# nickgreenquist/cu2rec

Hardware: AMD Instinct MI355X
Metric: ratings/sec (SGD updates/sec) (higher is better)
Workload: dtype f32

## Files before the change

### cu2rec_amd/csrc/blocksolve.hip

```cpp
#include <hip/hip_runtime.h>
#include <hip/hip_ext.h>

#include <algorithm>
#include <atomic>
#include <cmath>
#include <cstdlib>
#include <limits>
#include <mutex>
#include <string>
#include <utility>
#include <vector>

#include "blocksolve.hpp"
#include "hip_check.hpp"
#include "sgd_device.hpp"

namespace cu2rec {

namespace {

using namespace dev;

constexpr int kB = kBsLinks;
constexpr int kTabAdel = 0, kTabCdel = kBsTableStride, kTabApow = 2 * kBsTableStride, kTabCpow = 3 * kBsTableStride;
constexpr int kH = 32;
constexpr int kMS = 36;

typedef float f32x16 __attribute__((ext_vector_type(16)));
typedef float f32x4 __attribute__((ext_vector_type(4)));
typedef float f32x2 __attribute__((ext_vector_type(2)));
__device__ __forceinline__ f32x4 lds4(const float4 *p) { return *reinterpret_cast<const f32x4 *>(p); }
__device__ __forceinline__ f32x2 lo2(f32x4 v) { return __builtin_shufflevector(v, v, 0, 1); }
__device__ __forceinline__ f32x2 hi2(f32x4 v) { return __builtin_shufflevector(v, v, 2, 3); }
__device__ __forceinline__ f32x2 fma2(f32x2 a, f32x2 b, f32x2 c) { return __builtin_elementwise_fma(a, b, c); }
__device__ __forceinline__ f32x2 dup2(float v) { return f32x2{v, v}; }
typedef unsigned int u32x2 __attribute__((ext_vector_type(2)));

__device__ __forceinline__ unsigned ld_agent(const unsigned *p) {
    return __hip_atomic_load(p, __ATOMIC_RELAXED, __HIP_MEMORY_SCOPE_AGENT);
}
__device__ __forceinline__ unsigned long long ld_agent(const unsigned long long *p) {
    return __hip_atomic_load(p, __ATOMIC_RELAXED, __HIP_MEMORY_SCOPE_AGENT);
}

__device__ __forceinline__ float row_pair_sum(float v) {
    const u32x2 r = __builtin_amdgcn_permlane16_swap(__float_as_uint(v), __float_as_uint(v), false, false);
    return __uint_as_float(r.x) + __uint_as_float(r.y);
}

__device__ __forceinline__ float half_sum(float v) {
    const u32x2 r = __builtin_amdgcn_permlane32_swap(__float_as_uint(v), __float_as_uint(v), false, false);
    return __uint_as_float(r.x) + __uint_as_float(r.y);
}

__device__ __forceinline__ float lane_value(float v, int lane) {
    return __int_as_float(__builtin_amdgcn_readlane(__float_as_int(v), lane));
}

__device__ __forceinline__ int acc_row(int reg, int h) { return (reg & 3) + 8 * (reg >> 2) + 4 * h; }

__device__ __forceinline__ float4 zero4() { return make_float4(0.f, 0.f, 0.f, 0.f); }

__global__ void bs_tables_kernel(SgdHyper h, float *__restrict__ t) {
    const int k = threadIdx.x;
    if (k > 2 * kB) return;
    const double a = 1.0 - static_cast<double>(h.lr) * static_cast<double>(h.q_reg);
    const double c = 1.0 - static_cast<double>(h.lr) * static_cast<double>(h.ib_reg);
    double ak = 1.0, ck = 1.0;
    for (int i = 0; i < k; ++i) {
        ak *= a;
        ck *= c;
    }
    t[kTabAdel + k] = static_cast<float>(1.0 - ak);
    t[kTabCdel + k] = static_cast<float>(1.0 - ck);
    t[kTabApow + k] = static_cast<float>(ak);
    t[kTabCpow + k] = static_cast<float>(ck);
}

__device__ __forceinline__ int lower_bound_key(const uint32_t *__restrict__ keys, int n, uint32_t target) {
    int lo = 0, hi = n;
    while (lo < hi) {
        const int mid = (lo + hi) >> 1;
        if (keys[mid] < target) lo = mid + 1; else hi = mid;
    }
    return lo;
}

__global__ __launch_bounds__(256) void bs_plan_kernel(const uint32_t *__restrict__ keys, int n_active, int n_hot,
                                                      int item_bits, int max_blocks, const int *__restrict__ item_of_rank,
                                                      int *__restrict__ chain_begin, BsChainDesc *__restrict__ chains,
                                                      BsBlockDesc *__restrict__ blocks, int *__restrict__ walk_begin, size_t stride) {
    __shared__ int s_part[256];
    const int b = blockIdx.x, tid = threadIdx.x;
    const uint32_t *kb = keys + static_cast<size_t>(b) * stride;
    int *cb = chain_begin + static_cast<size_t>(b) * (n_hot + 1);
    BsChainDesc *cd = chains + static_cast<size_t>(b) * max(n_hot, 1);
    BsBlockDesc *bd = blocks + static_cast<size_t>(b) * max_blocks;
    for (int r = tid; r <= n_hot; r += 256) cb[r] = lower_bound_key(kb, n_active, static_cast<uint32_t>(r));
    __syncthreads();
    if (tid == 0) walk_begin[b] = cb[n_hot];
    const int per = (n_hot + 255) / 256;
    const int r0 = min(tid * per, n_hot), r1 = min(r0 + per, n_hot);
    int mine = 0;
    for (int r = r0; r < r1; ++r) mine += (cb[r + 1] - cb[r] + kB - 1) / kB;
    s_part[tid] = mine;
    __syncthreads();
    __shared__ int s_total;
    if (tid == 0) {
        int run = 0;
        for (int t = 0; t < 256; ++t) {
            const int v = s_part[t];
            s_part[t] = run;
            run += v;
        }
        s_total = run;
    }
    __syncthreads();
    int off = s_part[tid];
    for (int r = r0; r < r1; ++r) {
        const int begin = cb[r], len = cb[r + 1] - begin;
        cd[r] = BsChainDesc{begin, len, off, item_of_rank[r]};
        const int nb = (len + kB - 1) / kB;
        for (int m = 0; m < nb; ++m) bd[off + m] = BsBlockDesc{begin + kB * m, min(kB, len - kB * m), r, m};
        off += nb;
    }
    for (int g = s_total + tid; g < max_blocks; g += 256) bd[g] = BsBlockDesc{0, 0, 0, 0};
}

__device__ __forceinline__ bool chain_is_lookahead(const BsIteration &it, int chain, const BsChainDesc &cd) {
    const int nblk = (cd.len + kB - 1) / kB;
    return chain < it.la_ranks && nblk >= 2 && cd.blk0 + nblk <= it.la_cap;
}

__device__ __forceinline__ void gram_cross_block(const SgdArgs &a, const BsIteration &it, int g, float4 *smem) {
    const BsBlockDesc bd = it.blocks[g];
    if (bd.n_valid == 0 || bd.m == 0 || !chain_is_lookahead(it, bd.chain, it.chains[bd.chain])) return;
    const int wave = threadIdx.x >> 6, lane = threadIdx.x & 63, k = lane & 31, h = lane >> 5;
    const int rt = wave >> 1, ct = wave & 1;
    const int nslots = a.nslots, RS = nslots | 1, S0 = (nslots + 1) >> 1;
    float4 *tile_c = smem, *tile_p = smem + kB * RS;
    {
        const int xc = static_cast<int>(it.vals[bd.pos0 + min(lane, bd.n_valid - 1)] >> 32);
        const int xp = static_cast<int>(it.vals[bd.pos0 - kB + lane] >> 32);
        const int rsub = lane >> 3, cs = lane & 7;
        const int nch = (nslots + 7) >> 3;
        for (int c0 = 0; c0 < nch; c0 += 2) {
            float4 vc[2][2], vp[2][2];
#pragma unroll
            for (int pp = 0; pp < 2; ++pp) {
                const int src_lane = 16 * wave + 8 * pp + rsub;
                const float4 *sc = reinterpret_cast<const float4 *>(a.P + static_cast<size_t>(__shfl(xc, src_lane)) * a.ldp);
                const float4 *sp = reinterpret_cast<const float4 *>(a.P + static_cast<size_t>(__shfl(xp, src_lane)) * a.ldp);
#pragma unroll
                for (int c = 0; c < 2; ++c) {
                    vc[pp][c] = sc[min(8 * (c0 + c) + cs, nslots - 1)];
                    vp[pp][c] = sp[min(8 * (c0 + c) + cs, nslots - 1)];
                }
            }
#pragma unroll
            for (int pp = 0; pp < 2; ++pp) {
                const int row = 16 * wave + 8 * pp + rsub;
#pragma unroll
                for (int c = 0; c < 2; ++c) {
                    const int slot = 8 * (c0 + c) + cs;
                    if (slot < nslots) {
                        tile_c[row * RS + slot] = row < bd.n_valid ? vc[pp][c] : zero4();
                        tile_p[row * RS + slot] = vp[pp][c];
                    }
                }
            }
        }
    }
    __syncthreads();
    f32x16 acc;
#pragma unroll
    for (int i = 0; i < 16; ++i) acc[i] = 0.f;
    {
        const float4 *ra = tile_c + (kH * rt + k) * RS, *rb = tile_p + (kH * ct + k) * RS;
        for (int c = 0; c < S0; c += 2) {
            float4 va[2], vb[2];
#pragma unroll
            for (int i = 0; i < 2; ++i) {
                const int slot = h * S0 + c + i;
                const bool ok = c + i < S0 && slot < nslots;
                const float4 t0 = ra[min(slot, nslots - 1)], t1 = rb[min(slot, nslots - 1)];
                va[i] = ok ? t0 : zero4();
                vb[i] = ok ? t1 : zero4();
            }
#pragma unroll
            for (int i = 0; i < 2; ++i) {
                const float pa[4] = {va[i].x, va[i].y, va[i].z, va[i].w}, pb[4] = {vb[i].x, vb[i].y, vb[i].z, vb[i].w};
#pragma unroll
                for (int e = 0; e < 4; ++e) acc = __builtin_amdgcn_mfma_f32_32x32x2f32(pa[e], pb[e], acc, 0, 0, 0);
            }
        }
    }
    const float lr = a.h.lr;
    float *dst = it.Nbuf + static_cast<size_t>(g) * kBsCrossFloats;
    const int j = kH * ct + k;
#pragma unroll
    for (int reg = 0; reg < 16; ++reg) {
        const int i = kH * rt + acc_row(reg, h);
        const float fd = static_cast<float>(kB - 1 + i - j);
        const float v = lr * (__builtin_amdgcn_exp2f(fd * it.log2c) + __builtin_amdgcn_exp2f(fd * it.log2a) * acc[reg]);
        dst[i * kB + j] = i < bd.n_valid ? v : 0.f;
    }
    __syncthreads();
}

constexpr int kGramTabFloats = 2 * kB;
__host__ __device__ inline size_t gram_tile_float4s(int nslots) { return static_cast<size_t>(kB) * (nslots | 1); }

__device__ __forceinline__ void gram_block(const SgdArgs &a, const BsIteration &it, int g, float4 *bs_smem) {
    const int wave = threadIdx.x >> 6, lane = threadIdx.x & 63;
    const BsBlockDesc bd = it.blocks[g];
    if (bd.n_valid == 0) return;
    const int nslots = a.nslots, RS = nslots | 1;
    float4 *tile = bs_smem;
    float *Ms = reinterpret_cast<float *>(bs_smem);
    float *Ns = Ms + 2 * kH * kMS;
    float *tab = Ms + max(static_cast<int>(4 * gram_tile_float4s(nslots)), 5 * kH * kMS);
    float *basev = tab + kGramTabFloats;
    const bool mine = lane < bd.n_valid;
    const uint64_t val = it.vals[bd.pos0 + min(lane, bd.n_valid - 1)];
    const int x = static_cast<int>(val >> 32);
    if (wave == 3) {
        const float r0 = (__uint_as_float(static_cast<uint32_t>(val)) - a.global_bias) - a.user_bias[x];
        basev[lane] = mine ? r0 : 0.f;
        tab[lane] = it.tables[kTabApow + lane];
        tab[kB + lane] = it.tables[kTabCpow + lane];
    }
    const int rsub = lane >> 3, cs = lane & 7;
    const int nch = (nslots + 7) >> 3;
    for (int c0 = 0; c0 < nch; c0 += 4) {
        float4 v[2][4];
#pragma unroll
        for (int pp = 0; pp < 2; ++pp) {
            const int xr = __shfl(x, 16 * wave + 8 * pp + rsub);
            const float4 *src = reinterpret_cast<const float4 *>(a.P + static_cast<size_t>(xr) * a.ldp);
#pragma unroll
            for (int c = 0; c < 4; ++c) v[pp][c] = src[min(8 * (c0 + c) + cs, nslots - 1)];
        }
#pragma unroll
        for (int pp = 0; pp < 2; ++pp) {
            const int row = 16 * wave + 8 * pp + rsub;
#pragma unroll
            for (int c = 0; c < 4; ++c) {
                const int slot = 8 * (c0 + c) + cs;
                if (slot < nslots) tile[row * RS + slot] = row < bd.n_valid ? v[pp][c] : zero4();
            }
        }
    }
    __syncthreads();
    const int k = lane & 31, h = lane >> 5;
    f32x16 acc;
#pragma unroll
    for (int i = 0; i < 16; ++i) acc[i] = 0.f;
    if (wave < 3) {
        const int S0 = (nslots + 1) >> 1;
        const float4 *ra = tile + (wave == 1 ? kH + k : k) * RS, *rb = tile + (wave == 0 ? k : kH + k) * RS;
        for (int c = 0; c < S0; c += 2) {
            float4 va[2], vb[2];
#pragma unroll
            for (int i = 0; i < 2; ++i) {
                const int slot = h * S0 + c + i;
                const bool ok = c + i < S0 && slot < nslots;
                const float4 t0 = ra[min(slot, nslots - 1)], t1 = rb[min(slot, nslots - 1)];
                va[i] = ok ? t0 : zero4();
                vb[i] = ok ? t1 : zero4();
            }
#pragma unroll
            for (int i = 0; i < 2; ++i) {
                const float pa[4] = {va[i].x, va[i].y, va[i].z, va[i].w}, pb[4] = {vb[i].x, vb[i].y, vb[i].z, vb[i].w};
#pragma unroll
                for (int e = 0; e < 4; ++e) acc = __builtin_amdgcn_mfma_f32_32x32x2f32(pa[e], pb[e], acc, 0, 0, 0);
            }
        }
    }
    __syncthreads();
    if (wave < 3) {
        const float lr = a.h.lr;
        const int K = (wave == 0 ? 0 : kH) + k;
        const int J0 = (wave == 1 ? kH : 0) + 4 * h;
        const bool row_ok = K < bd.n_valid;
        float *dst = Ns + (wave * kH + k) * kMS + 4 * h;
#pragma unroll
        for (int m = 0; m < 4; ++m) {
            f32x4 out;
#pragma unroll
            for (int e = 0; e < 4; ++e) {
                const int d = K - 1 - (J0 + 8 * m + e);
                const float fd = static_cast<float>(d);
                const float v = lr * (__builtin_amdgcn_exp2f(fd * it.log2c) + __builtin_amdgcn_exp2f(fd * it.log2a) * acc[4 * m + e]);
                out[e] = d >= 0 && row_ok ? v : 0.f;
            }
            *reinterpret_cast<f32x4 *>(dst + 8 * m) = out;
        }
    }
    __syncthreads();
    if (wave == 0) {
    float m[kH];
    {
        const float *Nh = Ns + h * kH * kMS;
        float4 cur[8], nxt[8];
        m[0] = k == 0 ? 1.f : 0.f;
        cur[0] = *reinterpret_cast<const float4 *>(Nh + kMS);
#pragma unroll
        for (int kk = 1; kk < kH; ++kk) {
            if (kk + 1 < kH) {
#pragma unroll
                for (int i4 = 0; i4 < (kk + 4) / 4; ++i4) nxt[i4] = *reinterpret_cast<const float4 *>(Nh + (kk + 1) * kMS + 4 * i4);
            }
            __builtin_amdgcn_sched_barrier(0);
            float s[4] = {kk == k ? 1.f : 0.f, 0.f, 0.f, 0.f};
#pragma unroll
            for (int i4 = 0; i4 < (kk + 3) / 4; ++i4) {
                const float nv[4] = {cur[i4].x, cur[i4].y, cur[i4].z, cur[i4].w};
#pragma unroll
                for (int e = 0; e < 4; ++e)
                    if (4 * i4 + e < kk) s[e] = __builtin_fmaf(-nv[e], m[4 * i4 + e], s[e]);
            }
            m[kk] = (s[0] + s[1]) + (s[2] + s[3]);
            __builtin_amdgcn_sched_barrier(0);
            if (kk + 1 < kH) {
#pragma unroll
                for (int i4 = 0; i4 < (kk + 4) / 4; ++i4) cur[i4] = nxt[i4];
            }
        }
    }
#pragma unroll
    for (int kk = 0; kk < kH; ++kk) Ms[(h * kH + kk) * kMS + k] = m[kk];
    __builtin_amdgcn_wave_barrier();
    f32x16 tacc, macc;
#pragma unroll
    for (int i = 0; i < 16; ++i) tacc[i] = macc[i] = 0.f;
    {
        const float4 *arow = reinterpret_cast<const float4 *>(Ns + (2 * kH + k) * kMS + 16 * h);
#pragma unroll
        for (int t4 = 0; t4 < 4; ++t4) {
            const float4 a4 = arow[t4];
            const float av[4] = {a4.x, a4.y, a4.z, a4.w};
#pragma unroll
            for (int e = 0; e < 4; ++e)
                tacc = __builtin_amdgcn_mfma_f32_32x32x2f32(av[e], Ms[(16 * h + 4 * t4 + e) * kMS + k], tacc, 0, 0, 0);
        }
        const float *mrow = Ms + (kH + k) * kMS + 4 * h;
#pragma unroll
        for (int t4 = 0; t4 < 4; ++t4) {
            const float4 a4 = *reinterpret_cast<const float4 *>(mrow + 8 * t4);
            const float av[4] = {a4.x, a4.y, a4.z, a4.w};
#pragma unroll
            for (int e = 0; e < 4; ++e) macc = __builtin_amdgcn_mfma_f32_32x32x2f32(av[e], tacc[4 * t4 + e], macc, 0, 0, 0);
        }
    }
#pragma unroll
    for (int reg = 0; reg < 16; ++reg) Ns[acc_row(reg, h) * kMS + k] = -macc[reg];
    }
    __syncthreads();
    float *rec = it.Mbuf + static_cast<size_t>(g) * kBsRecFloats;
    {
        const int t = threadIdx.x, row = t >> 3, c4 = t & 7;
        const float *src[3] = {Ms, Ns, Ms + kH * kMS};
#pragma unroll
        for (int q = 0; q < 3; ++q) *reinterpret_cast<f32x4 *>(rec + q * kH * kH + 4 * t) = *reinterpret_cast<const f32x4 *>(src[q] + row * kMS + 4 * c4);
        if (t < kB / 4) *reinterpret_cast<f32x4 *>(rec + kBsFactorFloats + 4 * t) = *reinterpret_cast<const f32x4 *>(basev + 4 * t);
    }
}

__global__ __launch_bounds__(256, 4) void bs_gram_kernel(SgdArgs a, BsIteration it) {
    extern __shared__ float4 bs_smem[];
    const int g = static_cast<int>(blockIdx.x) - it.la_grid;
    __builtin_amdgcn_s_setprio(2);
    struct Through {
        unsigned long long *count;
        __device__ ~Through() {
            if (count && threadIdx.x == 0)
                __hip_atomic_fetch_add(count + 16 * (blockIdx.x & 31), 1ull, __ATOMIC_RELAXED, __HIP_MEMORY_SCOPE_AGENT);
        }
    } through_count{it.gram_done};
    if (g < 0) {
        const BsChainDesc last = it.chains[it.la_ranks - 1];
        const int la_end = min(last.blk0 + (last.len + kB - 1) / kB, it.la_cap);
        for (int gb = g + it.la_grid; gb < la_end; gb += it.la_grid) gram_cross_block(a, it, gb, bs_smem);
        return;
    }
    gram_block(a, it, g, bs_smem);
}

constexpr int kSolTabStride = kB + 1, kSolTabFloats = 4 * kSolTabStride;
constexpr int kSolTabAdel = 0, kSolTabCdel = kSolTabStride, kSolTabApow = 2 * kSolTabStride, kSolTabCpow = 3 * kSolTabStride;
constexpr int kRing = 2;
constexpr int kDepth = 4;

template <int N>
struct Stage {
    f32x4 rows[N];
    f32x4 m4[3];
    float base;
    uint64_t next_val;
};

__host__ __device__ inline int solve_slot_f4(int nslots) { return kB * (nslots | 1) + 3 * kH * kMS / 4; }

__host__ __device__ inline size_t solve_lds_bytes(int nslots, int sw) {
    return (static_cast<size_t>(kRing) * solve_slot_f4(nslots) + 4 * sw + 8 + 2 * kB + 8 * kB / 4 + (kSolTabFloats + 3) / 4 + 8 + 1) * 16;
}

__device__ __forceinline__ void solvers_meet(unsigned *meet, unsigned target, int lane) {
    __builtin_amdgcn_fence(__ATOMIC_RELEASE, "workgroup");
    if (lane == 0) __hip_atomic_fetch_add(meet, 1u, __ATOMIC_RELAXED, __HIP_MEMORY_SCOPE_WORKGROUP);
    while (__hip_atomic_load(meet, __ATOMIC_RELAXED, __HIP_MEMORY_SCOPE_WORKGROUP) < target) __builtin_amdgcn_s_sleep(1);
    __builtin_amdgcn_fence(__ATOMIC_ACQUIRE, "workgroup");
}

template <int SW>
__device__ __forceinline__ void solve_chain(const SgdArgs &a, const BsIteration &it, float4 *bs_smem, const BsChainDesc &cd) {
    const int begin = cd.begin, len = cd.len;
    if (len <= 0) return;
    const int nblk = (len + kB - 1) / kB;
    const int g0 = cd.blk0;
    const int nslots = a.nslots, RS = nslots | 1;
    const int S4 = solve_slot_f4(nslots);
    const bool long_chain = nblk > kDepth;
    const int n_intervals = long_chain ? (nblk + kDepth - 1) / kDepth * kDepth : kDepth;
    float4 *smem = bs_smem;
    const int tid = threadIdx.x;

    if (tid >= 256) {
        __builtin_amdgcn_s_setprio(2);
        constexpr int NLT = SW;
        const int lt = tid - 256, tr = lt >> 2, tp = lt & 3;
        auto load_val = [&](int t) -> uint64_t { return it.vals[begin + min(kB * t + tr, len - 1)]; };
        auto issue_rows = [&](Stage<NLT> &s, int t, uint64_t val) {
            s.next_val = load_val(t + kDepth);
            const f32x4 *row = reinterpret_cast<const f32x4 *>(a.P + static_cast<size_t>(static_cast<uint32_t>(val >> 32)) * a.ldp);
#pragma unroll
            for (int i = 0; i < NLT; ++i) s.rows[i] = row[min(tp + 4 * i, nslots - 1)];
        };
        auto issue_rec = [&](Stage<NLT> &s, int t) {
            const float *rec = it.Mbuf + static_cast<size_t>(g0 + min(t, nblk - 1)) * kBsRecFloats;
            const f32x4 *mg = reinterpret_cast<const f32x4 *>(rec);
#pragma unroll
            for (int q = 0; q < 3; ++q) s.m4[q] = mg[q * 256 + lt];
            s.base = rec[kBsFactorFloats + (lt & 63)];
        };
        auto issue = [&](Stage<NLT> &s, int t, uint64_t val) {
            issue_rows(s, t, val);
            issue_rec(s, t);
        };
        auto commit = [&](const Stage<NLT> &s, int t) {
            f32x4 *sl = reinterpret_cast<f32x4 *>(smem + (t % kRing) * S4);
            const bool rv = kB * t + tr < len;
            const f32x4 z = {0.f, 0.f, 0.f, 0.f};
#pragma unroll
            for (int i = 0; i < NLT; ++i) {
                const int slot = tp + 4 * i;
                if (slot < nslots) sl[tr * RS + slot] = rv ? s.rows[i] : z;
            }
            f32x4 *mt = sl + kB * RS;
#pragma unroll
            for (int q = 0; q < 3; ++q) {
                const int item = q * 256 + lt;
                mt[(item >> 3) * (kMS / 4) + (item & 7)] = s.m4[q];
            }
            if (lt < kB) reinterpret_cast<float *>(mt)[lt * kMS + kH] = kB * t + lt < len ? s.base : 0.f;
        };
        Stage<NLT> st[kDepth];
        if (long_chain) {
            uint64_t v[kDepth];
#pragma unroll
            for (int t = 0; t < kDepth; ++t) v[t] = load_val(t);
#pragma unroll
            for (int t = 0; t < kDepth; ++t) issue(st[t], t, v[t]);
            commit(st[0], 0);
            issue(st[0], kDepth, st[0].next_val);
            __syncthreads();
            for (int m0 = 0; m0 < n_intervals; m0 += kDepth) {
#pragma unroll
                for (int u = 0; u < kDepth; ++u) {
                    const int m = m0 + u;
                    Stage<NLT> &s = st[(u + 1) % kDepth];
                    commit(s, m + 1);
                    issue(s, m + 1 + kDepth, s.next_val);
                    __syncthreads();
                }
            }
        } else {
            uint64_t v[kDepth];
#pragma unroll
            for (int t = 0; t < kDepth; ++t) v[t] = load_val(min(t, nblk - 1));
#pragma unroll
            for (int t = 0; t < kDepth; ++t)
                if (t < nblk) issue(st[t], t, v[t]);
            commit(st[0], 0);
            __syncthreads();
#pragma unroll
            for (int u = 0; u < kDepth; ++u) {
                if (u + 1 < kDepth && u + 1 < nblk) commit(st[(u + 1) % kDepth], u + 1);
                __syncthreads();
            }
        }
        return;
    }

    __builtin_amdgcn_s_setprio(3);
    const int w = tid >> 6, k = tid & 63;
    constexpr int NP = (SW + 7) / 8;
    float4 *qrow = smem + kRing * S4;
    float4 *dpart = qrow + 4 * SW + 8;
    float4 *epart = dpart + kB;
    float *rbuf = reinterpret_cast<float *>(epart + kB) + w * kB;
    float *wbuf = reinterpret_cast<float *>(epart + kB) + (4 + w) * kB;
    float *tab = reinterpret_cast<float *>(epart + kB) + 8 * kB;
    float4 *zrow = reinterpret_cast<float4 *>(tab) + (kSolTabFloats + 3) / 4;
    unsigned *meet = reinterpret_cast<unsigned *>(zrow + 8);
    if (w == 0) {
        for (int i = k; i < kSolTabFloats; i += 64) tab[i] = it.tables[(i / kSolTabStride) * kBsTableStride + i % kSolTabStride];
        if (k < 8) zrow[k] = zero4();
        if (k == 0) *meet = 0u;
    }
    unsigned met = 0;
    const int y = cd.item;
    const int sl = k & 7, kg = k >> 3;
    f32x4 q4[NP];
    const f32x4 *qsrc = reinterpret_cast<const f32x4 *>(a.Q + static_cast<size_t>(y) * a.ldq);
#pragma unroll
    for (int p = 0; p < NP; ++p) {
        const int sq = 8 * p + sl, slot = w * SW + sq;
        const f32x4 v = qsrc[min(slot, nslots - 1)];
        q4[p] = sq < SW && slot < nslots ? v : f32x4{0.f, 0.f, 0.f, 0.f};
        if (kg == 0 && sq < SW) *reinterpret_cast<f32x4 *>(qrow + slot) = q4[p];
    }
    float b = a.item_bias[y];
    const float lr = a.h.lr;
    const int kr = k & 31;
    const bool upper = k >= kH;
    __syncthreads();
    for (int m = 0; m < n_intervals; ++m) {
        const bool live = m < nblk;
        const int n = min(kB, len - kB * m);
        const float4 *tile = smem + (m % kRing) * S4;
        const float *Mt = reinterpret_cast<const float *>(tile + kB * RS);
        float base = 0.f, adel_k = 0.f, cdel_k = 0.f, apr = 0.f, cpr = 0.f, adel_n = 0.f, cdel_n = 0.f;
        f32x4 mq[4];
        if (live) {
            const float4 *mrow = w < 2 ? reinterpret_cast<const float4 *>(Mt + ((upper ? kH : 0) + kr) * kMS + 16 * w)
                                       : (upper ? reinterpret_cast<const float4 *>(Mt + (2 * kH + kr) * kMS + 16 * (w - 2)) : zrow);
#pragma unroll
            for (int t = 0; t < 4; ++t) mq[t] = lds4(mrow + t);
            base = Mt[k * kMS + kH];
            const int back = max(n - 1 - k, 0);
            adel_k = tab[kSolTabAdel + k], cdel_k = tab[kSolTabCdel + k];
            apr = tab[kSolTabApow + back], cpr = tab[kSolTabCpow + back];
            adel_n = tab[kSolTabAdel + n], cdel_n = tab[kSolTabCdel + n];
            const float4 *prow = tile + k * RS;
            f32x4 pv[SW], qv[SW];
#pragma unroll
            for (int i = 0; i < SW; ++i) {
                pv[i] = lds4(prow + min(w * SW + i, nslots - 1));
                qv[i] = lds4(qrow + w * SW + i);
            }
            f32x2 dacc[2] = {dup2(0.f), dup2(0.f)};
#pragma unroll
            for (int i = 0; i < SW; ++i) {
                dacc[0] = fma2(lo2(pv[i]), lo2(qv[i]), dacc[0]);
                dacc[1] = fma2(hi2(pv[i]), hi2(qv[i]), dacc[1]);
            }
            const f32x2 ds = dacc[0] + dacc[1];
            reinterpret_cast<float *>(dpart)[4 * k + w] = ds.x + ds.y;
        }
        met += 4;
        solvers_meet(meet, met, k);
        if (live) {
            const f32x4 d4 = lds4(dpart + k);
            const float d = (d4.x + d4.y) + (d4.z + d4.w);
            const float rhs = k < n ? (base - (b - cdel_k * b)) - (d - adel_k * d) : 0.f;
            rbuf[k] = rhs;
            __builtin_amdgcn_wave_barrier();
            const float4 *rv = reinterpret_cast<const float4 *>(rbuf) + 4 * w;
            f32x2 eacc[2] = {dup2(0.f), dup2(0.f)};
#pragma unroll
            for (int t = 0; t < 4; ++t) {
                const f32x4 r4 = lds4(rv + t);
                eacc[0] = fma2(lo2(mq[t]), lo2(r4), eacc[0]);
                eacc[1] = fma2(hi2(mq[t]), hi2(r4), eacc[1]);
            }
            const f32x2 es = eacc[0] + eacc[1];
            reinterpret_cast<float *>(epart)[4 * k + w] = es.x + es.y;
        }
        met += 4;
        solvers_meet(meet, met, k);
        if (live) {
            const f32x4 e4 = lds4(epart + k);
            const float e = (e4.x + e4.y) + (e4.z + e4.w);
            if (w == 0) {
                const float e0 = k < n ? e : 0.f;
                const f32x4 e4v = {e0, dpp_move<0x55>(e0), dpp_move<0xAA>(e0), dpp_move<0xFF>(e0)};
                if ((k & 3) == 0) {
                    float *dst = it.ebuf + static_cast<size_t>(g0 + m) * kB + k;
                    *reinterpret_cast<f32x4 *>(dst) = e4v;
                }
            }
            wbuf[k] = k < n ? lr * apr * e : 0.f;
            const float bs = row_sum16(k < n ? lr * cpr * e : 0.f);
            b = (b - cdel_n * b) + ((lane_value(bs, 0) + lane_value(bs, 16)) + (lane_value(bs, 32) + lane_value(bs, 48)));
            __builtin_amdgcn_wave_barrier();
            float *qdst = it.qstart + static_cast<size_t>(g0 + m) * a.ldq;
            const float4 *wv = reinterpret_cast<const float4 *>(wbuf) + 2 * kg;
#pragma unroll
            for (int p = 0; p < NP; ++p) {
                const int sq = 8 * p + sl, slot = w * SW + sq;
                const bool ok = sq < SW && slot < nslots;
                if (ok && kg == 0) *reinterpret_cast<f32x4 *>(qdst + 4 * slot) = q4[p];
                const float4 *colp = tile + (8 * kg) * RS + min(slot, nslots - 1);
                f32x4 tb[8], wb[2];
#pragma unroll
                for (int i = 0; i < 8; ++i) tb[i] = lds4(colp + i * RS);
                wb[0] = lds4(wv), wb[1] = lds4(wv + 1);
                f32x2 ulo = dup2(0.f), uhi = dup2(0.f);
#pragma unroll
                for (int i = 0; i < 8; ++i) {
                    const f32x2 ww = dup2(wb[i >> 2][i & 3]);
                    ulo = fma2(ww, lo2(tb[i]), ulo);
                    uhi = fma2(ww, hi2(tb[i]), uhi);
                }
                float u[4] = {ulo.x, ulo.y, uhi.x, uhi.y};
#pragma unroll
                for (int c = 0; c < 4; ++c) {
                    u[c] += __int_as_float(__builtin_amdgcn_update_dpp(0, __float_as_int(u[c]), 0x128, 0xf, 0xf, false));
                    u[c] = half_sum(row_pair_sum(u[c]));
                }
                const f32x4 qo = q4[p];
                q4[p] = ok ? f32x4{(qo.x - adel_n * qo.x) + u[0], (qo.y - adel_n * qo.y) + u[1], (qo.z - adel_n * qo.z) + u[2],
                                   (qo.w - adel_n * qo.w) + u[3]}
// ... 280 lines not shown
                    const f32x2 ww = dup2(r < 4 ? wb0[r & 3] : wb1[r & 3]);
                    ulo = fma2(ww, lo2(tb[pp][r]), ulo);
                    uhi = fma2(ww, hi2(tb[pp][r]), uhi);
                }
                float u[4] = {ulo.x, ulo.y, uhi.x, uhi.y};
#pragma unroll
                for (int e = 0; e < 4; ++e) {
                    u[e] += __int_as_float(__builtin_amdgcn_update_dpp(0, __float_as_int(u[e]), 0x128, 0xf, 0xf, false));
                    u[e] = half_sum(row_pair_sum(u[e]));
                }
                const f32x4 qo = q4[pp];
                q4[pp] = ok ? f32x4{(qo.x - adel_n * qo.x) + u[0], (qo.y - adel_n * qo.y) + u[1], (qo.z - adel_n * qo.z) + u[2],
                                    (qo.w - adel_n * qo.w) + u[3]}
                            : f32x4{0.f, 0.f, 0.f, 0.f};
                if (ok && kg == 0) *reinterpret_cast<f32x4 *>(qbuf + ((i + 1) & 1) * kLaQ4 + slot) = q4[pp];
            }
            la_post(sy, kSyC0 + c, static_cast<unsigned>(i + 1));
        }
        if (kg == 0) {
            f32x4 *qd = reinterpret_cast<f32x4 *>(a.Q + static_cast<size_t>(y) * a.ldq);
#pragma unroll
            for (int pp = 0; pp < NPW; ++pp) {
                const int slot = 8 * (2 * pp + c) + sl;
                if (slot < nslots) qd[slot] = q4[pp];
            }
        }
        return;
    }

    const int k = lane;
    for (int i = k; i < kBsTableFloats; i += 64) tab[i] = it.tables[i];
    if (k < 16) sy[k] = 0u;
    float b_cur = a.item_bias[y], b_prev = b_cur;
    asm volatile("" ::"v"(b_cur));
    __syncthreads();
    __builtin_amdgcn_s_setprio(3);
    const int kr = k & 31;
    const bool upper = k >= kH;
    f32x4 m4[16], n4[16];
    float base;
    auto take_record = [&](int i) {
        la_wait4(sy, kSyLdR, static_cast<unsigned>(i + 1), it);
        const float4 *rr = rring + (i % kLaRRing) * kLaRec4;
        const float *Mt = reinterpret_cast<const float *>(rr);
        const float4 *mlo = reinterpret_cast<const float4 *>(Mt + ((upper ? kH : 0) + kr) * kMS);
        const float4 *mhi = reinterpret_cast<const float4 *>(Mt + (2 * kH + kr) * kMS);
        const float4 *nrow = rr + 3 * kH * kMS / 4 + k * kLaNS4;
#pragma unroll
        for (int j = 0; j < 8; ++j) {
            m4[j] = lds4(mlo + j);
            const f32x4 hi = lds4(mhi + j);
            m4[8 + j] = upper ? hi : f32x4{0.f, 0.f, 0.f, 0.f};
        }
#pragma unroll
        for (int j = 0; j < 16; ++j) n4[j] = lds4(nrow + j);
        base = Mt[k * kMS + kH];
        la_post(sy, kSyR, static_cast<unsigned>(i + 1));
    };
    take_record(0);
    for (int i = 0; i < nblk; ++i) {
        const int n = min(kB, len - kB * i);
        f32x2 tacc[2] = {dup2(0.f), dup2(0.f)};
        if (i > 0) {
            const float4 *ev = reinterpret_cast<const float4 *>(ebl + ((i - 1) & 1) * kB);
            f32x4 e4[16];
#pragma unroll
            for (int j = 0; j < 16; ++j) e4[j] = lds4(ev + j);
            __builtin_amdgcn_sched_barrier(0);
#pragma unroll
            for (int j = 0; j < 16; ++j) {
                tacc[0] = fma2(lo2(n4[j]), lo2(e4[j]), tacc[0]);
                tacc[1] = fma2(hi2(n4[j]), hi2(e4[j]), tacc[1]);
            }
        }
        const f32x2 ts = tacc[0] + tacc[1];
        const float t0 = ts.x + ts.y;
        const int kd = i > 0 ? k + kB : k;
        const float adel_k = tab[kTabAdel + kd], cdel_k = tab[kTabCdel + kd];
        const float bsrc = i > 0 ? b_prev : b_cur;
        la_wait(sy, kSyG, static_cast<unsigned>(i + 1), it);
        const float gd = gbuf[(i & 1) * kB + k];
        const float pre = k < n ? (base - (bsrc - cdel_k * bsrc)) - (gd - adel_k * gd) : 0.f;
        tbuf[k] = pre - t0;
        asm volatile("" ::: "memory");
        __builtin_amdgcn_wave_barrier();
        f32x2 eacc[2] = {dup2(0.f), dup2(0.f)};
        {
            const float4 *tv = reinterpret_cast<const float4 *>(tbuf);
            f32x4 t4[16];
#pragma unroll
            for (int j = 0; j < 16; ++j) t4[j] = lds4(tv + j);
            __builtin_amdgcn_sched_barrier(0);
#pragma unroll
            for (int j = 0; j < 16; ++j) {
                eacc[0] = fma2(lo2(m4[j]), lo2(t4[j]), eacc[0]);
                eacc[1] = fma2(hi2(m4[j]), hi2(t4[j]), eacc[1]);
            }
        }
        const f32x2 es = eacc[0] + eacc[1];
        const float e = k < n ? es.x + es.y : 0.f;
        const int back = max(n - 1 - k, 0);
        ebl[(i & 1) * kB + k] = e;
        wbuf[(i & 1) * kB + k] = k < n ? lr * tab[kTabApow + back] * e : 0.f;
        la_post(sy, kSyE, static_cast<unsigned>(i + 1));
        it.ebuf[static_cast<size_t>(g0 + i) * kB + k] = e;
        if (i + 1 < nblk) take_record(i + 1);
        const float bs = row_sum16(k < n ? lr * tab[kTabCpow + back] * e : 0.f);
        const float cdel_n = tab[kTabCdel + n];
        const float b_next = (b_cur - cdel_n * b_cur) + ((lane_value(bs, 0) + lane_value(bs, 16)) + (lane_value(bs, 32) + lane_value(bs, 48)));
        b_prev = b_cur;
        b_cur = b_next;
    }
    if (k == 0) a.item_bias[y] = b_cur;
}

__device__ __forceinline__ void await_iteration_end(const BsIteration &it) {
    const unsigned long long t0 = wall_clock64();
    unsigned polls = 0;
    while (it.side_seq && ld_agent(it.side_seq) < it.side_target) {
        __builtin_amdgcn_s_sleep(8);
        if ((++polls & 63u) == 0) {
            if (ld_agent(it.status) != 0u) break;
            if (wall_clock64() - t0 > 15ull * it.wait_ticks) {
                __hip_atomic_store(it.status, 1u, __ATOMIC_RELAXED, __HIP_MEMORY_SCOPE_AGENT);
                break;
            }
        }
    }
}

template <int SW>
__global__ __launch_bounds__(512) void bs_solve_kernel(SgdArgs a, BsIteration it) {
    extern __shared__ float4 bs_smem[];
    if (it.gram_done && threadIdx.x == 0)
        __hip_atomic_fetch_add(it.solve_started, 1ull, __ATOMIC_RELAXED, __HIP_MEMORY_SCOPE_AGENT);
    const int chain = blockIdx.x;
    const BsChainDesc cd = it.chains[chain];
    if constexpr (SW <= 8) {
        if (chain_is_lookahead(it, chain, cd)) {
            chain_lookahead<(4 * SW < kLaMaxSlots ? 4 * SW : kLaMaxSlots)>(a, it, bs_smem, cd);
            return;
        }
    }
    solve_chain<SW>(a, it, bs_smem, cd);
}

constexpr int kUpdMaxWaves = (4 * kBsMaxSlots + 63) / 64;

__device__ __forceinline__ void update_block(const SgdArgs &a, const BsIteration &it, int g) {
    const int wave = threadIdx.x >> 6, lane = threadIdx.x & 63;
    const BsBlockDesc bd = it.blocks[g];
    if (bd.n_valid == 0) return;
    const bool mine = lane < bd.n_valid;
    const uint64_t val = it.vals[bd.pos0 + min(lane, bd.n_valid - 1)];
    const int x = static_cast<int>(val >> 32);
    const float lr = a.h.lr;
    const int ncols = 4 * a.nslots;
    const int col = 64 * wave + lane, colc = min(col, ncols - 1);
    const float qs = it.qstart[static_cast<size_t>(g) * a.ldq + colc];
    const float e_all = it.ebuf[static_cast<size_t>(g) * kB + lane];
    const float e = mine ? e_all : 0.f;
    float p[kB];
#pragma unroll
    for (int k = 0; k < kB; ++k) {
        const int xk = __builtin_amdgcn_readlane(x, k);
        p[k] = a.P[static_cast<size_t>(xk) * a.ldp + colc];
    }
    float q = qs;
    const float p_reg = a.h.p_reg, q_reg = a.h.q_reg;
#pragma unroll
    for (int k = 0; k < kB; ++k) {
        const float ek = lane_value(e, k);
        const float pk = p[k];
        p[k] = pk + lr * (ek * q - p_reg * pk);
        q = q + lr * (ek * pk - q_reg * q);
    }
#pragma unroll
    for (int k = 0; k < kB; ++k) asm volatile("" : "+v"(p[k]));
    __builtin_amdgcn_sched_barrier(0);
    if (col < ncols) {
#pragma unroll
        for (int k = 0; k < kB; ++k) {
            if (k < bd.n_valid) a.P[static_cast<size_t>(__builtin_amdgcn_readlane(x, k)) * a.ldp + col] = p[k];
        }
    }
    if (wave == 0 && mine) {
        const float ub = a.user_bias[x];
        a.user_bias[x] = ub + lr * (e - a.h.ub_reg * ub);
    }
}

__global__ __launch_bounds__(64 * kUpdMaxWaves) void bs_update_kernel(SgdArgs a, BsIteration it) {
    const int g = blockIdx.x;
    __builtin_amdgcn_s_setprio(2);
    if (g == it.launch_blocks) {
        if (threadIdx.x == 0) await_iteration_end(it);
        return;
    }
    for (int blk = g; blk < it.max_blocks; blk += it.launch_blocks) {
        if (it.blocks[blk].n_valid == 0) break;
        update_block(a, it, blk);
    }
}

template <int SW>
void launch_solve_sw(const SgdArgs &a, const BsIteration &it, hipStream_t stream) {
    size_t lds = solve_lds_bytes(a.nslots, SW);
    if (it.la_ranks > 0) lds = std::max(lds, la_lds_bytes(a.nslots));
    ensure_max_dynamic_lds(reinterpret_cast<const void *>(bs_solve_kernel<SW>));
    hipLaunchKernelGGL((bs_solve_kernel<SW>), dim3(it.n_hot), dim3(512), lds, stream, a, it);
    const hipError_t err = hipGetLastError();
    if (err != hipSuccess)
        fail(CU2REC_EHIP, std::string("bs_solve_kernel launch failed: ") + hipGetErrorString(err) + " (SW " + std::to_string(SW) +
                              ", chains " + std::to_string(it.n_hot) + ", LDS " + std::to_string(lds) + " bytes)");
}

}

namespace {
__global__ void bs_probe_wait_kernel(const unsigned *word, unsigned *result, unsigned long long ticks) {
    if (threadIdx.x != 0) return;
    const unsigned long long t0 = wall_clock64();
    unsigned seen = 0;
    for (;;) {
        if (ld_agent(word) != 0u) {
            seen = 1;
            break;
        }
        __builtin_amdgcn_s_sleep(8);
        if (wall_clock64() - t0 > ticks) break;
    }
    __hip_atomic_store(result, seen ? 1u : 2u, __ATOMIC_RELAXED, __HIP_MEMORY_SCOPE_AGENT);
}

__global__ void bs_probe_signal_kernel(unsigned *word) {
    if (threadIdx.x == 0) __hip_atomic_store(word, 1u, __ATOMIC_RELAXED, __HIP_MEMORY_SCOPE_AGENT);
}

bool probe_streams(hipStream_t waiter, hipStream_t signaller, unsigned *scratch) {
    CU2REC_HIP(hipMemsetAsync(scratch, 0, 64 * sizeof(unsigned), waiter));
    CU2REC_HIP(hipStreamSynchronize(waiter));
    CU2REC_HIP(hipStreamSynchronize(signaller));
    hipLaunchKernelGGL(bs_probe_wait_kernel, dim3(1), dim3(64), 0, waiter, scratch, scratch + 32, 1000000ull);
    hipLaunchKernelGGL(bs_probe_signal_kernel, dim3(1), dim3(64), 0, signaller, scratch);
    CU2REC_HIP(hipGetLastError());
    CU2REC_HIP(hipStreamSynchronize(waiter));
    CU2REC_HIP(hipStreamSynchronize(signaller));
    unsigned result = 0;
    CU2REC_HIP(hipMemcpy(&result, scratch + 32, sizeof(unsigned), hipMemcpyDeviceToHost));
    return result == 1u;
}

int topology(DeviceRuntime &r, hipStream_t stream, hipStream_t side) {
    if (r.topology >= 0) return r.topology;
    if (const char *env = std::getenv("CU2REC_BS_GATE")) {
        r.topology = std::atoi(env) != 0 ? DeviceRuntime::kTopologyDevice : DeviceRuntime::kTopologyEvents;
        r.topology_forced = true;
        r.topology_why = std::string("CU2REC_BS_GATE=") + env;
        return r.topology;
    }
    if (const char *pmc = std::getenv("ROCPROF_COUNTER_COLLECTION"))
        if (*pmc && std::string(pmc) != "0" && std::string(pmc) != "False" && std::string(pmc) != "false") {
            r.topology = DeviceRuntime::kTopologyEvents;
            r.topology_why = "a rocprofv3 counter pass (ROCPROF_COUNTER_COLLECTION) serialises kernels across streams";
            return r.topology;
        }
    const bool forward = probe_streams(stream, side, r.probe);
    const bool backward = forward && probe_streams(side, stream, r.probe);
    if (forward && backward) {
        r.topology = DeviceRuntime::kTopologyDevice;
        r.topology_why = "two-stream handshake probe passed in both directions";
    } else {
        r.topology = DeviceRuntime::kTopologyEvents;
        r.topology_why = std::string("two-stream handshake probe: a wait kernel on the ") + (forward ? "side" : "main") +
                         " stream was not reached by the other stream's signal kernel within 10 ms (the streams do not run side by side here)";
    }
    return r.topology;
}

unsigned long long wait_ticks() {
    static const unsigned long long ticks = [] {
        double sec = 2.0;
        if (const char *env = std::getenv("CU2REC_BS_WAIT_S")) sec = std::max(0.001, std::atof(env));
        return static_cast<unsigned long long>(sec * 1e8);
    }();
    return ticks;
}

#ifdef CU2REC_TEST_HOOKS
int dbg() {
    static const int bits = std::getenv("CU2REC_BS_DBG") ? std::atoi(std::getenv("CU2REC_BS_DBG")) : 0;
    return bits;
}
#else
constexpr int dbg() { return 0; }
#endif

__global__ void bs_gate_kernel(const unsigned long long *count, unsigned long long target, const unsigned long long *started,
                               unsigned long long started_target, unsigned long long wait_ticks) {
    const int lane = threadIdx.x;
    const unsigned long long t0 = wall_clock64();
    unsigned polls = 0;
    for (;;) {
        unsigned long long v = lane < 32 ? ld_agent(count + 16 * lane) : 0ull;
#pragma unroll
        for (int off = 16; off > 0; off >>= 1) v += __shfl_xor(v, off);
        const unsigned long long sum = __shfl(v, 0);
        const unsigned long long st = ld_agent(started);
        if (sum >= target && st >= started_target) break;
        __builtin_amdgcn_s_sleep(16);
        if ((++polls & 63u) == 0 && wall_clock64() - t0 > wait_ticks) break;
    }
}

__global__ void bs_signal_kernel(unsigned long long *word, unsigned long long value) {
    if (threadIdx.x == 0) __hip_atomic_store(word, value, __ATOMIC_RELAXED, __HIP_MEMORY_SCOPE_AGENT);
}

void launch_gram(const SgdArgs &a, const BsIteration &it, hipStream_t stream, hipEvent_t stop) {
    size_t gram_lds = std::max(static_cast<size_t>(kB) * (a.nslots | 1) * 16, static_cast<size_t>(5) * kH * kMS * 4) +
                      static_cast<size_t>(kGramTabFloats + kB) * 4;
    if (it.la_ranks > 0) gram_lds = std::max(gram_lds, static_cast<size_t>(2) * kB * (a.nslots | 1) * 16);
    ensure_max_dynamic_lds(reinterpret_cast<const void *>(bs_gram_kernel));
    const int grid = it.max_blocks + (it.la_ranks > 0 ? it.la_grid : 0);
    if (stop) hipExtLaunchKernelGGL(bs_gram_kernel, dim3(grid), dim3(256), static_cast<uint32_t>(gram_lds), stream, nullptr, stop, 0, a, it);
    else hipLaunchKernelGGL(bs_gram_kernel, dim3(grid), dim3(256), gram_lds, stream, a, it);
    CU2REC_HIP(hipGetLastError());
}

void launch_solve(const SgdArgs &a, const BsIteration &it, hipStream_t stream) {
    const int sw = (a.nslots + 3) / 4;
    if (sw <= 1) launch_solve_sw<1>(a, it, stream);
    else if (sw <= 2) launch_solve_sw<2>(a, it, stream);
    else if (sw <= 4) launch_solve_sw<4>(a, it, stream);
    else if (sw <= 7) launch_solve_sw<7>(a, it, stream);
    else if (sw <= 8) launch_solve_sw<8>(a, it, stream);
    else if (sw <= 12) launch_solve_sw<12>(a, it, stream);
    else if (sw <= 16) launch_solve_sw<16>(a, it, stream);
    else fail(CU2REC_EUNSUPPORTED, "block-solve mode is compiled for n_factors <= 252");
}

void launch_update(const SgdArgs &a, const BsIteration &it, hipStream_t stream) {
    const int nwaves = (4 * a.nslots + 63) / 64;
    hipLaunchKernelGGL(bs_update_kernel, dim3(it.launch_blocks + (it.side_seq ? 1 : 0)), dim3(64 * nwaves), 0, stream, a, it);
    CU2REC_HIP(hipGetLastError());
}

std::atomic<int> g_lookahead{-1};
std::atomic<float> g_min_rate{-2.f};
constexpr float kDefaultRate = 240.f;

float min_rate_state() {
    float cur = g_min_rate.load();
    if (cur == -2.f) {
        float init = -1.f;
        if (const char *env = std::getenv("CU2REC_BLOCKSOLVE_RATE")) init = std::max(0.01f, static_cast<float>(std::atof(env)));
        g_min_rate.compare_exchange_strong(cur, init);
        cur = g_min_rate.load();
    }
    return cur;
}
}

int blocksolve_lookahead_blocks(int blocks) {
    int prev = g_lookahead.load();
    if (prev < 0) {
        const char *env = std::getenv("CU2REC_BLOCKSOLVE_LOOKAHEAD");
        const int init = env ? std::max(0, std::atoi(env)) : 24;
        g_lookahead.compare_exchange_strong(prev, init);
        prev = g_lookahead.load();
    }
    if (blocks >= 0) g_lookahead.store(blocks);
    return prev;
}

float blocksolve_min_rate(float rate) {
    const float prev = min_rate_state();
    if (rate > 0.f) g_min_rate.store(rate);
    else if (rate < 0.f) g_min_rate.store(-1.f);
    return prev > 0.f ? prev : -1.f;
}

int blocksolve_hot_items(const std::vector<double> &rate, int n_active, int rank_limit) {
    const float state = min_rate_state();
    float min_rate = state > 0.f ? state : kDefaultRate;
    const int n_cols = static_cast<int>(rate.size());
    if (state <= 0.f) {
        min_rate = std::max(30.f, min_rate * static_cast<float>(n_active) / 131072.f);
        if (n_cols > 0 && n_active <= 131072 / 4 && rate[0] < 350.0) min_rate = rate[0] >= 150.0 ? 60.f : std::numeric_limits<float>::infinity();
    }
    int n = 0;
    while (n < n_cols && rate[n] >= min_rate) ++n;
    return std::min(n, rank_limit);
}

BlockSolve::BlockSolve(int n_hot_, const std::vector<double> &rate, double hot_rate, int n_active_, int item_bits_, int max_batch_,
                       const int *item_of_rank_)
    : n_hot(n_hot_), n_active(n_active_), item_bits(item_bits_), max_batch(max_batch_), item_of_rank(item_of_rank_) {
    max_blocks = n_active / kBsLinks + n_hot + 1;
    const double bound = (hot_rate + 8.0 * std::sqrt(hot_rate) + 64.0) / kBsLinks + n_hot + 1;
    launch_blocks = std::max(1, bound >= static_cast<double>(max_blocks) ? max_blocks : static_cast<int>(bound));
    if (dbg() & 512) launch_blocks = std::min(3, max_blocks);
    const int la_min = blocksolve_lookahead_blocks(-1);
    double la_blocks = 0.0;
    while (la_min > 0 && la_ranks < n_hot && rate[la_ranks] >= static_cast<double>(la_min) * kBsLinks) {
        la_blocks += std::ceil(rate[la_ranks] / kBsLinks) + 1.0;
        ++la_ranks;
    }
    if (la_ranks > 0) la_cap = std::min(max_blocks, static_cast<int>(la_blocks * 1.25) + 4 * la_ranks + 8);
    for (int slot = 0; slot < 2; ++slot) {
        chain_begin[slot].allocate(static_cast<size_t>(max_batch) * (n_hot + 1));
        walk_begin[slot].allocate(max_batch);
        chains[slot].allocate(static_cast<size_t>(max_batch) * n_hot);
        blocks[slot].allocate(static_cast<size_t>(max_batch) * max_blocks);
    }
    tables.allocate(kBsTableFloats);
    Mbuf.allocate(static_cast<size_t>(max_blocks) * kBsRecFloats);
    ebuf.allocate(static_cast<size_t>(max_blocks) * kBsLinks);
    solve_started.allocate(16);
    solve_started.zero();
    gram_done.allocate(32 * 16);
    gram_done.zero();
    side_seq.allocate(16);
    side_seq.zero();
    if (la_cap > 0) Nbuf.allocate(static_cast<size_t>(la_cap) * kBsCrossFloats);
}

BlockSolve::~BlockSolve() {
    if (upd) (void)hipStreamDestroy(upd);
    for (hipEvent_t e : {ev_call, ev_upd, ev_gram})
        if (e) (void)hipEventDestroy(e);
}

void BlockSolve::plan(int slot, const uint32_t *sk, int nb, size_t stride, hipStream_t sched) {
    hipLaunchKernelGGL(bs_plan_kernel, dim3(nb), dim3(256), 0, sched, sk, n_active, n_hot, item_bits, max_blocks, item_of_rank,
                       chain_begin[slot].ptr, chains[slot].ptr, blocks[slot].ptr, walk_begin[slot].ptr, stride);
}

void BlockSolve::begin(const SgdArgs &a, hipStream_t stream) {
    if (a.nslots < 1 || a.nslots > kBsMaxSlots) fail(CU2REC_EUNSUPPORTED, "block-solve mode is compiled for n_factors <= 252");
    const bool same = tables_valid && tables_for.lr == a.h.lr && tables_for.q_reg == a.h.q_reg && tables_for.ib_reg == a.h.ib_reg;
    if (!same) {
        hipLaunchKernelGGL(bs_tables_kernel, dim3(1), dim3(192), 0, stream, a.h, tables.ptr);
        tables_for = a.h;
        tables_valid = true;
    }
    if (qstart_ld != a.ldq) {
        CU2REC_HIP(hipStreamSynchronize(stream));
        qstart.allocate(static_cast<size_t>(max_blocks) * a.ldq);
        qstart_ld = a.ldq;
    }
    if (!upd) {
        CU2REC_HIP(hipStreamCreateWithFlags(&upd, hipStreamNonBlocking));
        for (hipEvent_t *e : {&ev_call, &ev_upd, &ev_gram}) CU2REC_HIP(hipEventCreateWithFlags(e, hipEventDisableTiming));
    }
    unsigned *status = nullptr;
    {
        std::lock_guard<std::mutex> lock(device_runtime_mutex());
        DeviceRuntime &r = device_runtime();
        device_join = topology(r, stream, upd) == DeviceRuntime::kTopologyDevice;
        status = r.status + DeviceRuntime::kBlocksolveWord;
        host_status = r.host_status + 1;
    }
    CU2REC_HIP(hipEventRecord(ev_call, stream));
    CU2REC_HIP(hipStreamWaitEvent(upd, ev_call, 0));
    const bool la_on = la_ranks > 0 && la_supported(a.nslots);
    it = BsIteration{};
    it.n_active = n_active;
    it.n_hot = n_hot;
    it.item_mask = (1u << item_bits) - 1u;
    it.item_of_rank = item_of_rank;
    it.tables = tables.ptr;
    it.log2a = static_cast<float>(std::log2(1.0 - static_cast<double>(a.h.lr) * static_cast<double>(a.h.q_reg)));
    it.log2c = static_cast<float>(std::log2(1.0 - static_cast<double>(a.h.lr) * static_cast<double>(a.h.ib_reg)));
    it.Mbuf = Mbuf.ptr;
    it.ebuf = ebuf.ptr;
    it.qstart = qstart.ptr;
    it.max_blocks = max_blocks;
    it.launch_blocks = launch_blocks;
    it.la_ranks = la_on ? la_ranks : 0;
    it.la_cap = la_cap;
    it.la_grid = la_on ? la_cap : 0;
    it.Nbuf = Nbuf.ptr;
    it.status = status;
    it.solve_started = solve_started.ptr;
    it.wait_ticks = wait_ticks();
    if (device_join) {
        it.gram_done = gram_done.ptr;
        it.side_seq = side_seq.ptr;
    }
    upd_pending = false;
}

void BlockSolve::iteration(const SgdArgs &a, int slot, int b, const uint32_t *keys, const uint64_t *vals, bool last, hipStream_t stream,
                           const SideChains &side) {
    it.keys = keys;
    it.vals = vals;
    it.chains = chains[slot].ptr + static_cast<size_t>(b) * n_hot;
    it.blocks = blocks[slot].ptr + static_cast<size_t>(b) * max_blocks;
    it.walk_begin = walk_begin[slot].ptr + b;
    it.side_target = device_join ? side_seq_host + 1 : 0;
    if (upd_pending) CU2REC_HIP(hipStreamWaitEvent(stream, ev_upd, 0));
    launch_gram(a, it, stream, device_join ? nullptr : ev_gram);
    if (device_join) gram_done_target += static_cast<unsigned long long>(max_blocks + it.la_grid);
    else CU2REC_HIP(hipStreamWaitEvent(upd, ev_gram, 0));
    launch_solve(a, it, stream);
    if (device_join) {
        started_total += static_cast<unsigned long long>(n_hot);
        hipLaunchKernelGGL(bs_gate_kernel, dim3(1), dim3(64), 0, upd, gram_done.ptr, gram_done_target + ((dbg() & 32) ? (1ull << 40) : 0ull),
                           solve_started.ptr, started_total, it.wait_ticks);
        CU2REC_HIP(hipGetLastError());
    }
    side(upd, !device_join || last ? ev_upd : nullptr);
    if (device_join) {
        ++side_seq_host;
        if (!(dbg() & 16)) {
            hipLaunchKernelGGL(bs_signal_kernel, dim3(1), dim3(64), 0, upd, side_seq.ptr, side_seq_host);
            CU2REC_HIP(hipGetLastError());
        }
    }
    launch_update(a, it, stream);
    upd_pending = !device_join;
}

void BlockSolve::join(hipStream_t stream) {
    CU2REC_HIP(hipStreamWaitEvent(stream, ev_upd, 0));
    upd_pending = false;
}

void BlockSolve::end(hipStream_t stream) {
    CU2REC_HIP(hipMemcpyAsync(host_status, it.status, sizeof(unsigned), hipMemcpyDeviceToHost, stream));
}

}
```

Before: 1.777 billion.

## Invert triangular blocks via 16x16 diagonal solves and MFMA off-diagonal update

Replaces the per-lane sequential forward substitution over the full kH-sized unit lower-triangular matrix with a block approach. Each quarter-wave inverts a 16x16 diagonal block, and the off-diagonal block is then formed with two 16x16x4 MFMA products (-M22*N21*M11). This shortens the serial dependency chain and moves work onto the matrix cores. Separately, the gate kernel folds the 'started' load into the same lane-parallel load and polls with a shorter sleep, trading more memory polling for lower wake-up latency.

After: 1.773 billion (median of 3 runs). Within noise of the previous version (-0.2%).

```diff
diff --git a/cu2rec_amd/csrc/blocksolve.hip b/cu2rec_amd/csrc/blocksolve.hip
--- a/cu2rec_amd/csrc/blocksolve.hip
+++ b/cu2rec_amd/csrc/blocksolve.hip
@@ -299,20 +299,22 @@
     }
     __syncthreads();
     if (wave == 0) {
-    float m[kH];
     {
-        const float *Nh = Ns + h * kH * kMS;
-        float4 cur[8], nxt[8];
-        m[0] = k == 0 ? 1.f : 0.f;
-        cur[0] = *reinterpret_cast<const float4 *>(Nh + kMS);
-#pragma unroll
-        for (int kk = 1; kk < kH; ++kk) {
-            if (kk + 1 < kH) {
-#pragma unroll
-                for (int i4 = 0; i4 < (kk + 4) / 4; ++i4) nxt[i4] = *reinterpret_cast<const float4 *>(Nh + (kk + 1) * kMS + 4 * i4);
+        const int qd = lane >> 4, jd = lane & 15, bdiag = qd & 1;
+        float *Mx = Ms + (qd >> 1) * kH * kMS;
+        const float *Nb = Ns + (qd >> 1) * kH * kMS + 16 * bdiag * kMS + 16 * bdiag;
+        float m[16];
+        float4 cur[4], nxt[4];
+        m[0] = jd == 0 ? 1.f : 0.f;
+        cur[0] = *reinterpret_cast<const float4 *>(Nb + kMS);
+#pragma unroll
+        for (int kk = 1; kk < 16; ++kk) {
+            if (kk + 1 < 16) {
+#pragma unroll
+                for (int i4 = 0; i4 < (kk + 4) / 4; ++i4) nxt[i4] = *reinterpret_cast<const float4 *>(Nb + (kk + 1) * kMS + 4 * i4);
             }
             __builtin_amdgcn_sched_barrier(0);
-            float s[4] = {kk == k ? 1.f : 0.f, 0.f, 0.f, 0.f};
+            float s[4] = {kk == jd ? 1.f : 0.f, 0.f, 0.f, 0.f};
 #pragma unroll
             for (int i4 = 0; i4 < (kk + 3) / 4; ++i4) {
                 const float nv[4] = {cur[i4].x, cur[i4].y, cur[i4].z, cur[i4].w};
@@ -322,14 +324,36 @@
             }
             m[kk] = (s[0] + s[1]) + (s[2] + s[3]);
             __builtin_amdgcn_sched_barrier(0);
-            if (kk + 1 < kH) {
+            if (kk + 1 < 16) {
 #pragma unroll
                 for (int i4 = 0; i4 < (kk + 4) / 4; ++i4) cur[i4] = nxt[i4];
             }
         }
-    }
-#pragma unroll
-    for (int kk = 0; kk < kH; ++kk) Ms[(h * kH + kk) * kMS + k] = m[kk];
+#pragma unroll
+        for (int kk = 0; kk < 16; ++kk) {
+            Mx[(16 * bdiag + kk) * kMS + 16 * bdiag + jd] = m[kk];
+            Mx[(16 * (1 - bdiag) + kk) * kMS + 16 * bdiag + jd] = 0.f;
+        }
+    }
+    __builtin_amdgcn_wave_barrier();
+    {
+        const int id = lane & 15, gd = lane >> 4;
+#pragma unroll
+        for (int X = 0; X < 2; ++X) {
+            float *Mx = Ms + X * kH * kMS;
+            const float *Nx = Ns + X * kH * kMS;
+            f32x4 t = {0.f, 0.f, 0.f, 0.f}, r = {0.f, 0.f, 0.f, 0.f};
+#pragma unroll
+            for (int c = 0; c < 4; ++c)
+                t = __builtin_amdgcn_mfma_f32_16x16x4f32(Nx[(16 + id) * kMS + 4 * c + gd], Mx[(4 * c + gd) * kMS + id], t, 0, 0, 0);
+            const float4 mb = *reinterpret_cast<const float4 *>(Mx + (16 + id) * kMS + 16 + 4 * gd);
+            const float mbv[4] = {mb.x, mb.y, mb.z, mb.w};
+#pragma unroll
+            for (int c = 0; c < 4; ++c) r = __builtin_amdgcn_mfma_f32_16x16x4f32(mbv[c], t[c], r, 0, 0, 0);
+#pragma unroll
+            for (int rr = 0; rr < 4; ++rr) Mx[(16 + 4 * gd + rr) * kMS + id] = -r[rr];
+        }
+    }
     __builtin_amdgcn_wave_barrier();
     f32x16 tacc, macc;
 #pragma unroll
@@ -1216,13 +1240,14 @@
     const unsigned long long t0 = wall_clock64();
     unsigned polls = 0;
     for (;;) {
-        unsigned long long v = lane < 32 ? ld_agent(count + 16 * lane) : 0ull;
+        const unsigned long long w = ld_agent(lane < 32 ? count + 16 * lane : started);
+        unsigned long long v = lane < 32 ? w : 0ull;
 #pragma unroll
         for (int off = 16; off > 0; off >>= 1) v += __shfl_xor(v, off);
         const unsigned long long sum = __shfl(v, 0);
-        const unsigned long long st = ld_agent(started);
+        const unsigned long long st = __shfl(w, 32);
         if (sum >= target && st >= started_target) break;
-        __builtin_amdgcn_s_sleep(16);
+        __builtin_amdgcn_s_sleep(2);
         if ((++polls & 63u) == 0 && wall_clock64() - t0 > wait_ticks) break;
     }
 }
```
